# edwardyehuang/iSeg

Measured on AMD Instinct MI355X. Metric: train_images_per_sec (ConvNeXt-T+ASPP 512x512 crop, fwd+bwd+AdamW, whole job), higher is better.
Workload: dtype bf16

## Files before the change

include/iseg_hip.h:

```cpp
#ifndef ISEG_HIP_H
#define ISEG_HIP_H

#include <stddef.h>
#include <stdint.h>

#ifdef __cplusplus
extern "C" {
#endif

#ifndef ISEG_HIP_STREAM_T
#define ISEG_HIP_STREAM_T
typedef struct ihipStream_t* iseg_stream_t;
#endif

#define ISEG_STATUS_OK 0
#define ISEG_STATUS_ARG (-1)
#define ISEG_STATUS_HIP (-2)
#define ISEG_STATUS_UNSUPPORTED (-3)
#define ISEG_STATUS_WORKSPACE (-4)

#define ISEG_DTYPE_F32 0
#define ISEG_DTYPE_BF16 1

#define ISEG_ACT_NONE 0
// ... 425 lines not shown
typedef struct iseg_conv_geom {
    int N, H, W, Cin, Cout, KH, KW, sh, sw, dh, dw, pt, pl, Ho, Wo, groups;
} iseg_conv_geom;
int iseg_conv2d_igemm_supported(const iseg_conv_geom* geom_h, int dtype);
size_t iseg_conv2d_igemm_workspace_bytes(const iseg_conv_geom* geom_h, int pass);
int iseg_conv2d_igemm_fwd(const void* x, const void* w, const float* bias, void* y, const iseg_conv_geom* geom_h, int dtype, void* ws,
                          size_t ws_bytes, iseg_stream_t stream);
int iseg_conv2d_igemm_fwd_kt_supported(const iseg_conv_geom* g, int dtype);
int iseg_conv2d_igemm_fwd_kt(const void* x, const void* wt, const float* bias, void* y, const iseg_conv_geom* g, int dtype, void* ws,
                             size_t ws_bytes, iseg_stream_t stream);
int iseg_conv2d_igemm_bwd_data(const void* dy, const void* w, void* dx, const iseg_conv_geom* geom_h, int dtype, void* ws, size_t ws_bytes,
                               iseg_stream_t stream);
int iseg_conv2d_igemm_bwd_weight(const void* x, const void* dy, float* dw, int accumulate, const iseg_conv_geom* geom_h, int dtype, void* ws,
                                 size_t ws_bytes, iseg_stream_t stream);

int iseg_convnext_mlp_supported(int C, int dtype);
size_t iseg_convnext_mlp_tiled_bytes(int C, int backward);
int iseg_convnext_mlp_prep(const float* W1, const float* W2, const float* gamma, void* fw_tiled, void* bw_tiled, int C,
                           iseg_stream_t stream);
int iseg_convnext_weight_prep_batched(const int64_t* table, int entries, int64_t max_elements, iseg_stream_t stream);
int iseg_convnext_mlp_fwd(const void* y2, const void* fw_tiled, const float* b1, const float* b2, const float* gamma,
                          const float* rowscale, int64_t rows_per_group, const void* residual, void* out, int64_t M, int C, int dtype,
                          iseg_stream_t stream);
int iseg_convnext_mlp_bwd(const void* y2, const void* dbr, const void* bw_tiled, const float* b1, void* g, void* dh, void* dy2,
                          int64_t M, int C, int dtype, iseg_stream_t stream);
int iseg_convnext_mlp_bwd_data(const void* y, const float* mean, const float* rstd, const float* ln_gamma, const float* ln_beta,
                               const void* dout, const float* rowscale, int64_t rows_per_group, const void* bw_tiled, const float* b1,
                               void* dy2, int64_t M, int C, int dtype, iseg_stream_t stream);

size_t iseg_convnext_mlp_bwd_data_ln_workspace_bytes(int64_t M, int C);
// ... 18 lines not shown
```

iseg_amd/_hip.py:

```python
import ctypes as C
import os

_HERE = os.path.dirname(os.path.abspath(__file__))
LIB_PATH = os.path.join(_HERE, "lib", "libiseg_hip.so")

F32, BF16 = 0, 1
ACT_NONE, ACT_RELU, ACT_GELU, ACT_GELU_GRAD, ACT_RELU_GRAD, ACT_MUL_AUX, ACT_SIGMOID, ACT_SWISH = 0, 1, 2, 3, 4, 5, 6, 7


class HipLibraryMissing(RuntimeError):
    pass


class HipCallError(RuntimeError):
    pass


class GemmArgs(C.Structure):
    _fields_ = [
        ("A", C.c_void_p), ("lda", C.c_int64), ("a_kcontig", C.c_int),
        ("B", C.c_void_p), ("ldb", C.c_int64), ("b_kcontig", C.c_int),
        ("D", C.c_void_p), ("ldd", C.c_int64),
        ("M", C.c_int64), ("N", C.c_int64), ("K", C.c_int64),
        ("in_dtype", C.c_int), ("out_dtype", C.c_int),
# ... 2 lines not shown
        ("aux", C.c_void_p), ("ldaux", C.c_int64),
        ("pre_out", C.c_void_p), ("ldp", C.c_int64),
        ("act", C.c_int), ("alpha", C.c_float), ("accumulate", C.c_int), ("split_k", C.c_int), ("a_act", C.c_int),
        ("colsum_out", C.c_void_p), ("colsum_accumulate", C.c_int), ("defer_reduce", C.c_int),
        ("batch", C.c_int), ("batch_inner", C.c_int),
        ("sa_outer", C.c_int64), ("sa_inner", C.c_int64), ("sb_outer", C.c_int64), ("sb_inner", C.c_int64),
        ("sd_outer", C.c_int64), ("sd_inner", C.c_int64),
        ("pre_deriv", C.c_int),
        ("b_group_rows", C.c_int64),
        ("b_group_stride", C.c_int64),
    ]


class ConvGeom(C.Structure):
    _fields_ = [(n, C.c_int) for n in ("N", "H", "W", "Cin", "Cout", "KH", "KW", "sh", "sw", "dh", "dw", "pt", "pl", "Ho", "Wo", "groups")]


_p, _i, _l, _f, _z, _u64 = C.c_void_p, C.c_int, C.c_int64, C.c_float, C.c_size_t, C.c_uint64

SIGNATURES = {
    "iseg_version": (_i, []),
    "iseg_last_error": (_z, [C.c_char_p, _z]),
    "iseg_gemm_splits": (_i, [C.POINTER(GemmArgs)]),
    "iseg_gemm_tn_pair_splits": (_i, [C.POINTER(GemmArgs), C.POINTER(GemmArgs)]),
    "iseg_gemm_tn_pair": (_i, [C.POINTER(GemmArgs), _p, _z, C.POINTER(GemmArgs), _p, _z, _p]),
    "iseg_gemm_slabs": (_i, [C.POINTER(GemmArgs)]),
    "iseg_gemm_variant": (_i, [C.POINTER(GemmArgs)]),
    "iseg_gemm_workspace_bytes": (_z, [C.POINTER(GemmArgs)]),
    "iseg_gemm": (_i, [C.POINTER(GemmArgs), _p, _z, _p]),
    "iseg_gemm_reduce": (_i, [C.POINTER(GemmArgs), _p, _z, _p]),
# ... 168 lines not shown
    "iseg_augment_channel_means": (_i, [_p, _i, _p, _p, _i, _i, _i, _p, _z, _p]),
    "iseg_augment_crop_batch": (_i, [_p, _i, _p, _p, _p, C.POINTER(C.c_float), C.POINTER(C.c_float), C.POINTER(C.c_float), _i, _p, _p, _i, _i, _i,
                                     _i, _i, _u64, _p]),
    "iseg_normalize_image": (_i, [_p, _p, _l, C.POINTER(C.c_float), C.POINTER(C.c_float), _p]),
    "iseg_projective_transform_batch": (_i, [_p, _p, _p, _p, _p, _p, _i, _i, _i, _i, _i, _f, C.POINTER(C.c_float), _i, _p]),
    "iseg_upsample_ce_supported": (_i, [_i, _i, _i, _i, _i]),
    "iseg_upsample_ce_workspace_bytes": (_z, [_i, _i, _i, _i, _i, _i]),
    "iseg_upsample_ce": (_i, [_p, _i, _p, _p, _i, _i, _i, _i, _i, _i, _i, _p, _f, _p, _f, _p, _p, _z, _p]),
    "iseg_conv2d_igemm_supported": (_i, [C.POINTER(ConvGeom), _i]),
    "iseg_conv2d_igemm_workspace_bytes": (_z, [C.POINTER(ConvGeom), _i]),
    "iseg_conv2d_igemm_fwd": (_i, [_p, _p, _p, _p, C.POINTER(ConvGeom), _i, _p, _z, _p]),
    "iseg_conv2d_igemm_fwd_kt": (_i, [_p, _p, _p, _p, C.POINTER(ConvGeom), _i, _p, _z, _p]),
    "iseg_conv2d_igemm_fwd_kt_supported": (_i, [C.POINTER(ConvGeom), _i]),
    "iseg_conv2d_igemm_bwd_data": (_i, [_p, _p, _p, C.POINTER(ConvGeom), _i, _p, _z, _p]),
    "iseg_conv2d_igemm_bwd_weight": (_i, [_p, _p, _p, _i, C.POINTER(ConvGeom), _i, _p, _z, _p]),
    "iseg_convnext_mlp_supported": (_i, [_i, _i]),
    "iseg_convnext_mlp_tiled_bytes": (_z, [_i, _i]),
    "iseg_convnext_mlp_prep": (_i, [_p, _p, _p, _p, _p, _i, _p]),
    "iseg_convnext_mlp_fwd": (_i, [_p, _p, _p, _p, _p, _p, _l, _p, _p, _l, _i, _i, _p]),
    "iseg_convnext_mlp_bwd": (_i, [_p, _p, _p, _p, _p, _p, _p, _l, _i, _i, _p]),
    "iseg_convnext_mlp_bwd_data": (_i, [_p, _p, _p, _p, _p, _p, _p, _l, _p, _p, _p, _l, _i, _i, _p]),
    "iseg_convnext_mlp_bwd_data_ln_workspace_bytes": (_z, [_l, _i]),
    "iseg_convnext_mlp_bwd_data_ln": (_i, [_p, _p, _p, _p, _p, _p, _p, _l, _p, _p, _p, _p, _p, _l, _i, _i, _p, _z, _p]),
    "iseg_convnext_weight_prep_batched": (_i, [_p, _i, _l, _p]),
    "iseg_convnext_mlp_fwd_ln": (_i, [_p, _p, _p, _f, _p, _p, _p, _p, _p, _p, _p, _l, _p, _p, _l, _i, _i, _p]),
    "iseg_convnext_mlp_wgrad_workspace_bytes": (_z, [_l, _i]),
    "iseg_convnext_mlp_wgrad": (_i, [_p, _p, _p, _p, _p, _p, _p, _l, _p, _p, _p, _p, _p, _p, _p, _p, _p, _p, _l, _i, _i, _p, _z, _p]),
    "iseg_sgd_momentum_step": (_i, [_p, _p, _p, _p, _p, _p, _p, _p, _f, _i, _p, _f, _p, _f, _l, _p]),
}

# ... 35 lines not shown
```

iseg_amd/csrc/conv_igemm.hip:

```cpp
#include <type_traits>

#include "gemm_impl.h"

using namespace iseg_mm;

int gemm_reduce(const iseg_gemm_args* g, const Epi& epi, float* slabs, int eff_split, int64_t slab_rows, hipStream_t stream);

namespace {

struct ConvP {
    const bf16_t* src;
    int Hs, Ws, Cs;
    int Hr, Wr;
    int Cg;
    int kw;
    int sh, sw, dh, dw, pt, pl;
    int groups;
};

struct PhaseP {
    int Hq, Wq;
    int a, b;
    int q0h, q0w;
    int Th, Tw;
// ... 4 lines not shown
struct PhaseTable {
    PhaseP ph[MAX_PHASES];
    int H, W, sh, sw, kw;
};
struct NoPhases {};

struct PhaseRows {
    int hw, wq, H, W, sh, sw, a, b;
    __device__ __forceinline__ int64_t operator()(int64_t m) const {
        const int n = (int)(m / hw), rem = (int)(m % hw);
        return ((int64_t)n * H + (rem / wq) * sh + a) * W + (rem % wq) * sw + b;
    }
};

constexpr int INVALID = -(1 << 28);

}

#include "conv_igemm_dma.h"

namespace {

__device__ __forceinline__ bf16x8 gather8(const ConvP& p, int nb, int ih, int iw, int c, bool ok) {
    bf16x8 v;
#pragma unroll
    for (int i = 0; i < 8; ++i) v[i] = (bf16_t)0.f;
    if (ok && ih >= 0 && ih < p.Hs && iw >= 0 && iw < p.Ws) v = *reinterpret_cast<const bf16x8*>(p.src + ((int64_t)(nb + ih * p.Ws + iw)) * p.Cs + c);
    return v;
}

// ... 72 lines not shown
                const int64_t row = n0 + r;
                bf16x8 v;
#pragma unroll
                for (int u = 0; u < 8; ++u) v[u] = (bf16_t)0.f;
                if (row < R && kk < Kend) {
                    const int ij = (int)(kk / cout_g), co = (int)(kk % cout_g);
                    const int tap = tap0 + (ij / tw) * tsh + (ij % tw) * tsw;
                    v = *reinterpret_cast<const bf16x8*>(wg + tap * tap_stride + row * ld + co);
                }
                this->regs[i] = v;
            }
        }
    }
};

template <int WM, int WN, int FM, int FN, int PASS, int BK, class TO>
__global__ __launch_bounds__(WM* WN * 64) void conv_igemm_kernel(ConvP p, const bf16_t* __restrict__ Bop, int64_t ldb, int64_t b_group_stride,
                                                                  int64_t tap_stride, TO* __restrict__ D, int64_t ldd, int64_t d_group_stride,
                                                                  int64_t M, int64_t N, int64_t K, int tiles_n, int ntiles,
                                                                  int64_t k_per_split, float* __restrict__ slabs, int64_t slab_group_stride,
                                                                  Epi epi, int vecD,
                                                                  typename std::conditional<PASS == 3, PhaseTable, NoPhases>::type phases) {
    constexpr bool AKC = PASS != 2, BKC = PASS == 1 || PASS == 3;
    constexpr int GPASS = PASS == 3 ? 1 : PASS;
    constexpr int NT = WM * WN * 64;
    constexpr int BM = WM * FM * 16, BN = WN * FN * 16;
    constexpr int TM = FM * 16, TN = FN * 16;
    constexpr int KS = BK / 32;
    using GA = TileGeom<BM, AKC, BK>;
    using GB = TileGeom<BN, BKC, BK>;
    constexpr int STAGE_ELEMS = GA::elems + GB::elems;
    constexpr int EPI_BYTES = WM * WN * 32 * (TN + 4) * 4;
    constexpr int LDS_BYTES = (STAGE_ELEMS * 2 > EPI_BYTES) ? STAGE_ELEMS * 2 : EPI_BYTES;
    __shared__ __attribute__((aligned(16))) char smem[LDS_BYTES];
    bf16_t* const lds = reinterpret_cast<bf16_t*>(smem);

    const int tid = threadIdx.x, lane = tid & 63, wid = tid >> 6;
    const int wm = wid / WN, wn = wid % WN;
    const int grp = blockIdx.z;
    const int coff = grp * p.Cg;
    Bop += grp * b_group_stride;
    D += grp * d_group_stride;
    if (slabs) slabs += grp * slab_group_stride;
    if (epi.bias) epi.bias += grp * N;

    int t, ksplit;
    int tw = p.kw, tap0 = 0, tsh = p.kw, tsw = 1;
    PhaseRows rows{};
    if constexpr (PASS == 3) {
        const PhaseP& ph = phases.ph[blockIdx.y];
        M = ph.M;
        K = ph.K;
        k_per_split = K;
        t = blockIdx.x;
        ksplit = 0;
        if ((int64_t)(t / tiles_n) * BM >= M) return;
        p.Hr = ph.Hq, p.Wr = ph.Wq, p.kw = ph.Tw, p.pt = ph.q0h, p.pl = ph.q0w;
        p.sh = p.sw = p.dh = p.dw = 1;
        tw = ph.Tw, tap0 = ph.tap0, tsh = phases.sh * phases.kw, tsw = phases.sw;
        rows = PhaseRows{ph.Hq * ph.Wq, ph.Wq, phases.H, phases.W, phases.sh, phases.sw, ph.a, ph.b};
    } else {
        tile_and_split(ntiles, t, ksplit);
    }
    const int tile_n = t % tiles_n, tile_m = t / tiles_n;
    const int64_t m0 = (int64_t)tile_m * BM, n0 = (int64_t)tile_n * BN;
    const int64_t kbeg = (int64_t)ksplit * k_per_split;
    const int64_t kend = (kbeg + k_per_split < K) ? kbeg + k_per_split : K;
    const int nk = (int)((kend - kbeg + BK - 1) / BK);

    f32x4 acc[FM][FN];
#pragma unroll
    for (int i = 0; i < FM; ++i)
#pragma unroll
        for (int j = 0; j < FN; ++j) acc[i][j] = f32x4{0.f, 0.f, 0.f, 0.f};

    GatherStager<BM, NT, BK, GPASS> sa;
    typename std::conditional<BKC, TapWeightStager<BN, NT, BK>, Stager<BN, false, NT, BK>>::type sb;
    sa.prepare(p, m0, M, coff, tid);

    auto load_b = [&](int64_t k0) {
// ... 23 lines not shown
            for (int j = 0; j < FN; ++j) bfr[j] = read_frag<BN, BKC, BK>(lds + GA::elems, wn * TN + j * 16, ks, lane);
#pragma unroll
            for (int i = 0; i < FM; ++i)
#pragma unroll
                for (int j = 0; j < FN; ++j) acc[i][j] = __builtin_amdgcn_mfma_f32_16x16x32_bf16(bfr[j], af[i], acc[i][j], 0, 0, 0);
        }
        __syncthreads();
        if (more) {
            sa.store(lds, tid);
            sb.store(lds + GA::elems, tid);
            __syncthreads();
        }
    }
    if constexpr (PASS == 3) tile_epilogue<WM, WN, FM, FN, TO, PhaseRows>(acc, smem, D, ldd, M, N, m0, n0, wm, wn, wid, lane, nullptr, epi, false, vecD, 0, rows);
    else tile_epilogue<WM, WN, FM, FN, TO>(acc, smem, D, ldd, M, N, m0, n0, wm, wn, wid, lane, slabs, epi, false, vecD, ksplit);
}

struct Problem {
    int64_t M, N, K;
    ConvP p;
    const bf16_t* B;
    int64_t ldb, b_group_stride, tap_stride;
    void* D;
    int64_t ldd, d_group_stride;
    int out_dtype;
    const float* bias;
    int accumulate;
    int groups;
};

// ... 287 lines not shown
    q.M = (int64_t)g->KH * g->KW * cg;
    q.N = og;
    q.K = (int64_t)g->N * g->Ho * g->Wo;
    q.p = ConvP{(const bf16_t*)x, g->H, g->W, g->Cin, g->Ho, g->Wo, cg, g->KW, g->sh, g->sw, g->dh, g->dw, g->pt, g->pl, g->groups};
    q.B = (const bf16_t*)dy;
    q.ldb = g->Cout;
    q.b_group_stride = og;
    q.D = dw;
    q.ldd = g->Cout;
    q.d_group_stride = og;
    q.out_dtype = ISEG_F32;
    q.accumulate = accumulate;
    q.groups = g->groups;
    return run<2, float>(q, ws, ws_bytes, stream, "iseg_conv2d_igemm_bwd_weight");
}
```

iseg_amd/csrc/conv_igemm_dma.h:

```cpp
#pragma once
#include "gemm_dma.h"

namespace {

__device__ uint4 conv_zero_page[8];

template <int WM, int WN, int NS, int PASS, class TO>
__global__ __launch_bounds__(WM* WN * 64) void conv_igemm_dma_kernel(ConvP p, const bf16_t* __restrict__ Bop, int64_t ldb, int64_t tap_stride,
                                                                      TO* __restrict__ D, int64_t ldd, int64_t M, int64_t N, int64_t K,
                                                                      int tiles_n, int ntiles, int64_t k_per_split, float* __restrict__ slabs,
                                                                      Epi epi) {
    using namespace iseg_mm;
    constexpr int FN = 4;
    constexpr int NW = WM * WN;
    constexpr int BM = WM * 64, BN = WN * FN * 16;
    constexpr int PIECES = (BM + BN) / 8, PPW = PIECES / NW;
    static_assert(PIECES % NW == 0, "stage pieces must divide over the wavefronts");
    constexpr int STAGE = (BM + BN) * 128;
    extern __shared__ __attribute__((aligned(1024))) char smem[];

    const int tid = threadIdx.x, lane = tid & 63, wid = tid >> 6;
    const int wm = wid / WN, wn = wid % WN;
    int t, ksplit;
    tile_and_split(ntiles, t, ksplit);
    const int64_t m0 = (int64_t)(t / tiles_n) * BM, n0 = (int64_t)(t % tiles_n) * BN;
    const int64_t kbeg = (int64_t)ksplit * k_per_split;
    const int64_t kend = (kbeg + k_per_split < K) ? kbeg + k_per_split : K;
    const int nk = (int)((kend - kbeg) / 64);
// ... 14 lines not shown
                a1[q] = (rem % p.Wr) * p.sw - p.pl;
            } else {
                a0[q] = rem / p.Wr + p.pt;
                a1[q] = rem % p.Wr + p.pl;
            }
            a2[q] = (int64_t)n * p.Hs * p.Ws;
        } else {
            const int rb = r - BM;
            int64_t row = n0 + rb;
            row = row < N ? row : N - 1;
            a0[q] = ((lane & 7) ^ b_key(rb)) * 8;
            a1[q] = 0;
            a2[q] = row * ldb;
        }
    }
    auto issue = [&](int stage, int kt) {
        const int64_t k0 = kbeg + (int64_t)kt * 64;
        const int tap = (int)(k0 / p.Cg), c0 = (int)(k0 % p.Cg);
        const int ti = tap / p.kw, tj = tap % p.kw;
#pragma unroll
        for (int q = 0; q < PPW; ++q) {
            const int r = (wid + q * NW) * 8 + rsub;
            const bf16_t* src;
            if (r < BM) {
                const int chunk = ((lane & 7) ^ (r & 7)) * 8;
                int ih, iw;
                bool ok;
                if (PASS == 0) {
                    ih = a0[q] + ti * p.dh;
                    iw = a1[q] + tj * p.dw;
                    ok = (unsigned)ih < (unsigned)p.Hs && (unsigned)iw < (unsigned)p.Ws;
                } else {
                    const int th = a0[q] - ti * p.dh, tw = a1[q] - tj * p.dw;
                    ih = th / p.sh;
                    iw = tw / p.sw;
                    ok = th >= 0 && tw >= 0 && ih * p.sh == th && iw * p.sw == tw && ih < p.Hs && iw < p.Ws;
                }
                src = ok ? p.src + (a2[q] + (int64_t)ih * p.Ws + iw) * p.Cs + c0 + chunk : zero + chunk;
            } else if (PASS == 0) {
                src = Bop + a2[q] + k0 + a0[q];
            } else {
                src = Bop + (int64_t)tap * tap_stride + a2[q] + c0 + a0[q];
            }
            __builtin_amdgcn_global_load_lds((glb_void_ptr)src, (lds_void_ptr)(smem + stage * STAGE + (wid + q * NW) * 1024), 16, 0, 0);
        }
    };

    f32x4 acc[4][FN];
// ... 72 lines not shown
                for (int u = 0; u < 8; ++u) v[u] = acc[i][2 * h + (u >> 2)][u & 3];
                if (split) {
                    float* dst = slab + m * N + n;
                    *reinterpret_cast<float4*>(dst) = *reinterpret_cast<const float4*>(v);
                    *reinterpret_cast<float4*>(dst + 4) = *reinterpret_cast<const float4*>(v + 4);
                } else {
                    EpiPrefetch<TO> pf;
                    pf.load(epi, m, n, D, ldd);
                    epi_finish8<TO>(epi, v, pf, m, n, D, ldd);
                }
            }
        }
    }
}

}
```

iseg_amd/functional.py:

```python
import os

import torch
from torch.autograd import Function

from . import kernels as K
from . import nn
from . import dist


def _grad(p):
    if p.grad is None:
        p.grad = torch.zeros_like(p.data)
    return p.grad


def _c(t):
    return t if t.is_contiguous() else t.contiguous()


def _rows2d(t):
    C = t.shape[-1]
    if t.is_contiguous():
        return t.reshape(-1, C), C
    per16 = 16 // t.element_size()
# ... 398 lines not shown
    if groups == 1:
        return xc
    N, H, W, Cin = xc.shape
    out = torch.empty((N, H, W, Cin_g), dtype=xc.dtype, device=xc.device)
    K.copy2d(xc.reshape(-1, Cin)[:, g * Cin_g:], Cin, out.reshape(-1, Cin_g), Cin_g, N * H * W, Cin_g)
    return out


def conv2d(x, W, b=None, strides=(1, 1), dilation=(1, 1), padding="same", groups=1):
    if nn.dry_run():
        Ho, Wo, _, _ = _conv_geometry(x.shape[1], x.shape[2], W.shape[0], W.shape[1], tuple(strides), tuple(dilation), padding)
        return _dry((x.shape[0], Ho, Wo, W.shape[-1]), x, nn.compute_dtype())
    return _Conv2dFn.apply(x, W, b, tuple(strides), tuple(dilation), padding, int(groups))


class _DWConvFn(Function):
    @staticmethod
    def forward(ctx, x, W, b, dil):
        Kk, C = W.shape[0], W.shape[2]
        pad = (Kk - 1) * dil // 2
        xc = _c(x)
        y = K.dwconv2d(xc, W.data.reshape(Kk * Kk, C), b.data if b is not None else None, Kk, dil, pad, pad)
        ctx.W, ctx.b, ctx.dil, ctx.pad = W, b, dil, pad
        ctx.save_for_backward(xc)
        return y

    @staticmethod
    def backward(ctx, dy):
        (xc,) = ctx.saved_tensors
        W, b, dil, pad = ctx.W, ctx.b, ctx.dil, ctx.pad
# ... 2287 lines not shown
```

iseg_amd/kernels.py:

```python
import contextlib
import ctypes as C

import torch

from . import _hip
from ._hip import F32, BF16, ACT_NONE, ACT_RELU, ACT_GELU, ACT_GELU_GRAD, ACT_RELU_GRAD, ACT_MUL_AUX, ACT_SIGMOID, ACT_SWISH, GemmArgs

_DT = {torch.float32: F32, torch.bfloat16: BF16}


def dt(t):
    try:
        return _DT[t.dtype if isinstance(t, torch.Tensor) else t]
    except KeyError:
        raise TypeError(f"iseg_amd kernels support float32 and bfloat16 storage, got {t.dtype if isinstance(t, torch.Tensor) else t}")


def ptr(t):
    return None if t is None else t.data_ptr()


_DEVICE_INDEX = [None]


# ... 755 lines not shown
def conv2d_igemm_bwd_data(dy, w, geom):
    _require_cuda(dy, w)
    dx = torch.empty((geom.N, geom.H, geom.W, geom.Cin), dtype=dy.dtype, device=dy.device)
    ws, wsb = _conv_ws(geom, 1, dy.device)
    _hip.call("iseg_conv2d_igemm_bwd_data", ptr(dy), ptr(w), ptr(dx), C.byref(geom), dt(dy), ptr(ws), wsb, stream())
    return dx


def conv2d_igemm_bwd_weight(x, dy, dw, geom, accumulate=True):
    _require_cuda(x, dy, dw)
    ws, wsb = _conv_ws(geom, 2, x.device)
    _hip.call("iseg_conv2d_igemm_bwd_weight", ptr(x), ptr(dy), ptr(dw), int(accumulate), C.byref(geom), dt(x), ptr(ws), wsb, stream())
    return dw


def colsum(x, ldx, batch_stride, batch, rows, Cc, out, scale=1.0, accumulate=False):
    if Cc > 8192 and batch == 1 and scale == 1.0:
        L = _hip.lib()
        ws, wsb = workspace(L.iseg_colsum_wide_workspace_bytes(rows, Cc), x.device)
        _hip.check(L.iseg_colsum_wide(ptr(x), ldx, rows, Cc, ptr(out), int(accumulate), dt(x), ptr(ws), wsb, stream()), "iseg_colsum_wide")
        return out
    need = _hip.lib().iseg_colsum_workspace_bytes(batch, rows, Cc)
    ws, wsb = workspace(need, x.device)
    _hip.call("iseg_colsum", ptr(x), ldx, batch_stride, batch, rows, Cc, ptr(out), scale, int(accumulate), dt(x), ptr(ws), wsb,
              stream())
    return out


def accumulate_pair(src, n, dst0, dst1):
    if dst0 is None and dst1 is None:
# ... 892 lines not shown
```

iseg_amd/layers/aspp.py:

```python
from .. import functional as F
from ..nn import Layer
from .model_builder import ConvNormAct, ImageLevelBlock


class AtrousSpatialPyramidPooling(Layer):
    def __init__(self, filters=256, dilation_rates=[3, 6, 9], dilation_rates_multiplier=1, use_pixel_level=True,
                 use_image_level=True, name=None):
        super().__init__(name=name)
        self.filters = filters
        self.use_pixel_level = use_pixel_level
        self.use_image_level = use_image_level
        self.dilation_rates = list(dilation_rates)
        self.dilation_rates_multiplier = dilation_rates_multiplier

    def build(self, input_shape):
        if self.use_image_level:
            self.image_level_block = ImageLevelBlock(self.filters, name=f"{self.name}/image_level_block")
        if self.use_pixel_level:
            self.pixel_level_block = ConvNormAct(self.filters, (1, 1), name=f"{self.name}/pixel_level_block")
        convs = []
        for rate in self.dilation_rates:
            rate = rate * self.dilation_rates_multiplier
            convs.append(ConvNormAct(self.filters, (3, 3), dilation_rate=rate, name=f"{self.name}/asp_convs_{rate}"))
        import torch

        self.asp_convs = torch.nn.ModuleList(convs)
        self.built = True

    def call(self, inputs, training=None):
        if self._can_group(training):
            return self._call_grouped(inputs)
        branches = int(self.use_image_level) + int(self.use_pixel_level) + len(self.asp_convs)
        xs = list(F.fork(inputs, branches))
        blocks = ([self.image_level_block] if self.use_image_level else []) + ([self.pixel_level_block] if self.use_pixel_level else []) + \
            list(self.asp_convs)
        return F.concat([b(x, training=training) for b, x in zip(blocks, xs)])

    def _branch_blocks(self):
        blocks = []
        if self.use_image_level:
            blocks.append(self.image_level_block.convbnrelu)
        if self.use_pixel_level:
            blocks.append(self.pixel_level_block)
        return blocks + list(self.asp_convs)

    def _can_group(self, training):
        from .. import dist, nn
        from .base_layers import BatchNormalization

        if not (training and dist.active()) or nn.dry_run():
            return False
        for b in self._branch_blocks():
            if not (isinstance(b.bn, BatchNormalization) and b.bn.synchronized and b.bn.trainable and b.activation is F.relu and
                    b.dropout is None and b.bn.built):
                return False
        return True

    def _call_grouped(self, inputs):
        blocks = self._branch_blocks()
        xs = list(F.fork(inputs, len(blocks)))
        h, w = inputs.shape[1], inputs.shape[2]
        pre = []
        for i, b in enumerate(blocks):
            x = xs[i]
            if self.use_image_level and i == 0:
                x = F.global_avg_pool(x)
            pre.append(b.conv(x))
        outs = list(F.batch_norm_group(pre, [b.bn for b in blocks], relu=True))
        if self.use_image_level:
            outs[0] = F.broadcast_hw(outs[0], h, w)
        return F.concat(outs)
```

iseg_amd/layers/model_builder.py:

```python
import torch

from .. import functional as F
from .. import nn
from ..nn import Layer
from ..utils.common import resize_image
from .base_layers import Conv2D, Dropout, get_activation
from .normalizations import normalization


def get_training_value(training=None):
    if training is None:
        return False
    if isinstance(training, int):
        training = bool(training)
    return training


class ConvNormAct(Layer):
    def __init__(self, filters=256, kernel_size=1, dilation_rate=1, use_bn=True, activation="relu",
                 kernel_initializer="glorot_uniform", dropout_rate=0, dropout_before_bn=False, trainable=True, use_bias=False,
                 groups=1, conv_func=Conv2D, norm_func=normalization, name=None):
        super().__init__(trainable=trainable, name=name if name is not None else "ConvBnRelu")
        self.conv = conv_func(filters, kernel_size, padding="same", use_bias=use_bias, kernel_initializer=kernel_initializer,
                              dilation_rate=dilation_rate, groups=groups, trainable=trainable, name=f"{self.name}/conv")
        self.bn = None if not use_bn else norm_func(trainable=trainable, name=f"{self.name}/bn")
        self.activation = get_activation(activation)
        self.dropout = None
        self.dropout_before_bn = dropout_before_bn
        if dropout_rate > 0:
            self.dropout = Dropout(dropout_rate, name=f"{self.name}/dropout")

    def call(self, inputs, training=None):
        x = self.conv(inputs)
        should_dropout = (self.dropout is not None) and self.trainable
        if should_dropout and self.dropout_before_bn:
            x = self.dropout(x, training=training)
        act = self.activation
        if self.bn is not None:
            fuse = act is F.relu and hasattr(self.bn, "moving_mean")
            x = self.bn(x, training=training, fused_relu=True) if fuse else self.bn(x, training=training)
            if fuse:
                act = None
        if act is not None:
            x = act(x)
        if should_dropout and not self.dropout_before_bn:
            x = self.dropout(x, training=training)
        return x

# ... 134 lines not shown
```

Measured before the change: 2021.

## Fuse ASPP pixel-branch convolutions into single multi-branch igemm kernels

Adds a branch-table convolution API that runs all ASPP pixel-level and atrous convolutions sharing one input in a single kernel launch per pass. Forward launches one grid over the branches, backward-data sums all branches' taps into one joined K reduction with an optional fused residual, and backward-weight handles every branch in one launch. This is meant to cut launch count, repeated forks of the input, and separate dx accumulation across branches. The fused path only applies to bf16, bias-free, stride-1, same-padded convs with channel counts that are multiples of 64, and it adds new kernel code paths.

```diff
diff --git a/include/iseg_hip.h b/include/iseg_hip.h
--- a/include/iseg_hip.h
+++ b/include/iseg_hip.h
@@ -463,6 +463,29 @@
 int iseg_conv2d_igemm_bwd_weight(const void* x, const void* dy, float* dw, int accumulate, const iseg_conv_geom* geom_h, int dtype, void* ws,
                                  size_t ws_bytes, iseg_stream_t stream);
 
+#define ISEG_CONV_MAX_BRANCHES 4
+typedef struct iseg_conv_branch {
+    int KH, KW, dh, dw, pt, pl;
+    const void* wt;
+    const void* w;
+    const float* bias;
+    void* y;
+    int64_t ldy, y_col;
+    const void* dy;
+    int64_t lddy;
+    float* gw;
+} iseg_conv_branch;
+typedef struct iseg_conv_branches {
+    int N, H, W, Cin, Cout, count;
+    iseg_conv_branch b[ISEG_CONV_MAX_BRANCHES];
+} iseg_conv_branches;
+int iseg_conv2d_branches_supported(const iseg_conv_branches* t, int dtype);
+int iseg_conv2d_branches_fwd(const void* x, const iseg_conv_branches* t, int dtype, void* ws, size_t ws_bytes, iseg_stream_t stream);
+int iseg_conv2d_branches_bwd_data(const iseg_conv_branches* t, void* dx, const void* residual, int64_t ldr, int dtype, void* ws, size_t ws_bytes,
+                                  iseg_stream_t stream);
+int iseg_conv2d_branches_bwd_weight(const void* x, const iseg_conv_branches* t, int accumulate, int dtype, void* ws, size_t ws_bytes,
+                                    iseg_stream_t stream);
+
 int iseg_convnext_mlp_supported(int C, int dtype);
 size_t iseg_convnext_mlp_tiled_bytes(int C, int backward);
 int iseg_convnext_mlp_prep(const float* W1, const float* W2, const float* gamma, void* fw_tiled, void* bw_tiled, int C,
diff --git a/iseg_amd/_hip.py b/iseg_amd/_hip.py
--- a/iseg_amd/_hip.py
+++ b/iseg_amd/_hip.py
@@ -40,6 +40,19 @@
 
 class ConvGeom(C.Structure):
     _fields_ = [(n, C.c_int) for n in ("N", "H", "W", "Cin", "Cout", "KH", "KW", "sh", "sw", "dh", "dw", "pt", "pl", "Ho", "Wo", "groups")]
+
+
+CONV_MAX_BRANCHES = 4
+
+
+class ConvBranch(C.Structure):
+    _fields_ = [(n, C.c_int) for n in ("KH", "KW", "dh", "dw", "pt", "pl")] + [
+        ("wt", C.c_void_p), ("w", C.c_void_p), ("bias", C.c_void_p), ("y", C.c_void_p), ("ldy", C.c_int64), ("y_col", C.c_int64),
+        ("dy", C.c_void_p), ("lddy", C.c_int64), ("gw", C.c_void_p)]
+
+
+class ConvBranches(C.Structure):
+    _fields_ = [(n, C.c_int) for n in ("N", "H", "W", "Cin", "Cout", "count")] + [("b", ConvBranch * CONV_MAX_BRANCHES)]
 
 
 _p, _i, _l, _f, _z, _u64 = C.c_void_p, C.c_int, C.c_int64, C.c_float, C.c_size_t, C.c_uint64
@@ -238,6 +251,10 @@
     "iseg_conv2d_igemm_fwd_kt_supported": (_i, [C.POINTER(ConvGeom), _i]),
     "iseg_conv2d_igemm_bwd_data": (_i, [_p, _p, _p, C.POINTER(ConvGeom), _i, _p, _z, _p]),
     "iseg_conv2d_igemm_bwd_weight": (_i, [_p, _p, _p, _i, C.POINTER(ConvGeom), _i, _p, _z, _p]),
+    "iseg_conv2d_branches_supported": (_i, [C.POINTER(ConvBranches), _i]),
+    "iseg_conv2d_branches_fwd": (_i, [_p, C.POINTER(ConvBranches), _i, _p, _z, _p]),
+    "iseg_conv2d_branches_bwd_data": (_i, [C.POINTER(ConvBranches), _p, _p, _l, _i, _p, _z, _p]),
+    "iseg_conv2d_branches_bwd_weight": (_i, [_p, C.POINTER(ConvBranches), _i, _i, _p, _z, _p]),
     "iseg_convnext_mlp_supported": (_i, [_i, _i]),
     "iseg_convnext_mlp_tiled_bytes": (_z, [_i, _i]),
     "iseg_convnext_mlp_prep": (_i, [_p, _p, _p, _p, _p, _i, _p]),
diff --git a/iseg_amd/csrc/conv_igemm.hip b/iseg_amd/csrc/conv_igemm.hip
--- a/iseg_amd/csrc/conv_igemm.hip
+++ b/iseg_amd/csrc/conv_igemm.hip
@@ -42,6 +42,23 @@
 };
 
 constexpr int INVALID = -(1 << 28);
+
+struct BranchP {
+    const bf16_t* src;
+    const bf16_t* B;
+    void* D;
+    const float* bias;
+    int64_t ldb, ldd;
+    int Cs;
+    int kw, dh, dw, pt, pl;
+    int K;
+};
+constexpr int MAX_BRANCHES = ISEG_CONV_MAX_BRANCHES;
+struct BranchTable {
+    BranchP b[MAX_BRANCHES];
+    int count;
+};
+struct NoBranches {};
 
 }
 
@@ -144,13 +161,11 @@
     }
 };
 
-template <int WM, int WN, int FM, int FN, int PASS, int BK, class TO>
-__global__ __launch_bounds__(WM* WN * 64) void conv_igemm_kernel(ConvP p, const bf16_t* __restrict__ Bop, int64_t ldb, int64_t b_group_stride,
-                                                                  int64_t tap_stride, TO* __restrict__ D, int64_t ldd, int64_t d_group_stride,
-                                                                  int64_t M, int64_t N, int64_t K, int tiles_n, int ntiles,
-                                                                  int64_t k_per_split, float* __restrict__ slabs, int64_t slab_group_stride,
-                                                                  Epi epi, int vecD,
-                                                                  typename std::conditional<PASS == 3, PhaseTable, NoPhases>::type phases) {
+template <int WM, int WN, int FM, int FN, int PASS, int BK, class TO, bool RAGGED = false>
+__device__ __forceinline__ void conv_igemm_tile(ConvP p, const bf16_t* __restrict__ Bop, int64_t ldb, int64_t b_group_stride, int64_t tap_stride,
+                                                TO* __restrict__ D, int64_t ldd, int64_t d_group_stride, int64_t M, int64_t N, int64_t K, int tiles_n,
+                                                int ntiles, int64_t k_per_split, float* __restrict__ slabs, int64_t slab_group_stride, Epi epi,
+                                                int vecD, const typename std::conditional<PASS == 3, PhaseTable, NoPhases>::type& phases, int grp) {
     constexpr bool AKC = PASS != 2, BKC = PASS == 1 || PASS == 3;
     constexpr int GPASS = PASS == 3 ? 1 : PASS;
     constexpr int NT = WM * WN * 64;
@@ -167,7 +182,6 @@
 
     const int tid = threadIdx.x, lane = tid & 63, wid = tid >> 6;
     const int wm = wid / WN, wn = wid % WN;
-    const int grp = blockIdx.z;
     const int coff = grp * p.Cg;
     Bop += grp * b_group_stride;
     D += grp * d_group_stride;
@@ -194,6 +208,7 @@
     }
     const int tile_n = t % tiles_n, tile_m = t / tiles_n;
     const int64_t m0 = (int64_t)tile_m * BM, n0 = (int64_t)tile_n * BN;
+    if (RAGGED && m0 >= M) return;
     const int64_t kbeg = (int64_t)ksplit * k_per_split;
     const int64_t kend = (kbeg + k_per_split < K) ? kbeg + k_per_split : K;
     const int nk = (int)((kend - kbeg + BK - 1) / BK);
@@ -247,6 +262,26 @@
     }
     if constexpr (PASS == 3) tile_epilogue<WM, WN, FM, FN, TO, PhaseRows>(acc, smem, D, ldd, M, N, m0, n0, wm, wn, wid, lane, nullptr, epi, false, vecD, 0, rows);
     else tile_epilogue<WM, WN, FM, FN, TO>(acc, smem, D, ldd, M, N, m0, n0, wm, wn, wid, lane, slabs, epi, false, vecD, ksplit);
+}
+
+template <int WM, int WN, int FM, int FN, int PASS, int BK, class TO>
+__global__ __launch_bounds__(WM* WN * 64) void conv_igemm_kernel(ConvP p, const bf16_t* __restrict__ Bop, int64_t ldb, int64_t b_group_stride,
+                                                                  int64_t tap_stride, TO* __restrict__ D, int64_t ldd, int64_t d_group_stride,
+                                                                  int64_t M, int64_t N, int64_t K, int tiles_n, int ntiles,
+                                                                  int64_t k_per_split, float* __restrict__ slabs, int64_t slab_group_stride,
+                                                                  Epi epi, int vecD,
+                                                                  typename std::conditional<PASS == 3, PhaseTable, NoPhases>::type phases) {
+    conv_igemm_tile<WM, WN, FM, FN, PASS, BK, TO>(p, Bop, ldb, b_group_stride, tap_stride, D, ldd, d_group_stride, M, N, K, tiles_n, ntiles,
+                                                  k_per_split, slabs, slab_group_stride, epi, vecD, phases, blockIdx.z);
+}
+
+template <int WM, int WN, int FM, int FN, int BK>
+__global__ __launch_bounds__(WM* WN * 64) void conv_branches_wgrad_kernel(ConvP p, BranchTable tab, int64_t N, int64_t K, int tiles_n, int ntiles,
+                                                                           Epi epi, int vecD) {
+    const BranchP& br = tab.b[blockIdx.z];
+    p.kw = br.kw, p.dh = br.dh, p.dw = br.dw, p.pt = br.pt, p.pl = br.pl;
+    conv_igemm_tile<WM, WN, FM, FN, 2, BK, float, true>(p, br.B, br.ldb, 0, 0, (float*)br.D, br.ldd, 0, br.K, N, K, tiles_n, ntiles, K, nullptr, 0, epi,
+                                                        vecD, NoPhases{}, 0);
 }
 
 struct Problem {
@@ -564,3 +599,199 @@
     q.groups = g->groups;
     return run<2, float>(q, ws, ws_bytes, stream, "iseg_conv2d_igemm_bwd_weight");
 }
+
+namespace {
+
+bool branches_ok(const iseg_conv_branches* t) {
+    if (!t || t->count < 1 || t->count > MAX_BRANCHES || t->N <= 0 || t->H <= 0 || t->W <= 0 || t->Cin <= 0 || t->Cout <= 0) return false;
+    for (int i = 0; i < t->count; ++i) {
+        const iseg_conv_branch& b = t->b[i];
+        if (b.KH <= 0 || b.KW <= 0 || b.dh <= 0 || b.dw <= 0 || b.pt < 0 || b.pl < 0) return false;
+    }
+    return true;
+}
+
+ConvP branches_shared(const iseg_conv_branches* t, const void* src, int Cs, int Cg) {
+    return ConvP{(const bf16_t*)src, t->H, t->W, Cs, t->H, t->W, Cg, 1, 1, 1, 1, 1, 0, 0, 1};
+}
+
+struct DgradPlan {
+    bool big;
+    int nsplit;
+};
+DgradPlan branches_dgrad_plan(int64_t M, int64_t N, int64_t K) { return DgradPlan{M >= 256, conv_splits(M, N, K, 1)}; }
+
+iseg_conv_geom branches_joined_geom(const iseg_conv_branches* t) {
+    int taps = 0;
+    for (int i = 0; i < t->count; ++i) taps += t->b[i].KH * t->b[i].KW;
+    return iseg_conv_geom{t->N, t->H, t->W, t->Cin, t->Cout, 1, taps, 1, 1, 1, 1, 0, 0, t->H, t->W, 1};
+}
+
+template <int PASS, class Tile>
+void launch_branches_dma(Tile, const ConvP& p, const BranchTable& tab, int64_t ldb, int64_t tap_stride, bf16_t* D, int64_t ldd, int64_t M, int64_t N,
+                         int64_t K, int eff, int64_t kps, float* slabs, const Epi& epi, hipStream_t stream) {
+    constexpr int WM = Tile::WM, WN = Tile::WN, FN = Tile::FN, NS = Tile::NS;
+    constexpr int BM = WM * 64, BN = WN * FN * 16;
+    constexpr int lds = NS * (BM + BN) * 128;
+    const int tiles_m = (int)ceil_div64(M, BM), tiles_n = (int)ceil_div64(N, BN);
+    static const bool raised = [] {
+        return hipFuncSetAttribute(reinterpret_cast<const void*>(&conv_branches_dma_kernel<WM, WN, FN, NS, PASS>),
+                                   hipFuncAttributeMaxDynamicSharedMemorySize, lds) == hipSuccess;
+    }();
+    (void)raised;
+    hipLaunchKernelGGL((conv_branches_dma_kernel<WM, WN, FN, NS, PASS>), dim3(tiles_m * tiles_n, eff, PASS == 0 ? tab.count : 1), dim3(WM * WN * 64), lds,
+                       stream, p, tab, ldb, tap_stride, D, ldd, M, N, K, tiles_n, tiles_m * tiles_n, kps, slabs, epi);
+}
+struct BT256 { enum { WM = 4, WN = 2, FN = 4, NS = 3 }; };
+struct BT128 { enum { WM = 2, WN = 4, FN = 2, NS = 2 }; };
+
+}
+
+extern "C" int iseg_conv2d_branches_supported(const iseg_conv_branches* t, int dtype) {
+    if (!branches_ok(t) || dtype != ISEG_BF16) return 0;
+    if (t->Cin % 64 != 0 || t->Cout % 64 != 0) return 0;
+    const int64_t M = (int64_t)t->N * t->H * t->W;
+    return M >= 64 && M < (1ll << 31) / 8;
+}
+
+#define BRANCHES_COMMON(name)                                                                                                                  \
+    ISEG_REQUIRE(t, name ": null branch table");                                                                                              \
+    ISEG_REQUIRE(t->count >= 1 && t->count <= MAX_BRANCHES, name ": %d branches, the table holds 1 .. %d", t->count, MAX_BRANCHES);          \
+    ISEG_REQUIRE(branches_ok(t), name ": bad geometry");                                                                                      \
+    if (!iseg_conv2d_branches_supported(t, dtype)) {                                                                                          \
+        iseg_set_error(name ": needs bf16 storage, Cin and Cout multiples of 64 and at least 64 pixels (Cin %d, Cout %d, dtype %d)", t->Cin,  \
+                       t->Cout, dtype);                                                                                                       \
+        return ISEG_ERR_UNSUPPORTED;                                                                                                          \
+    }                                                                                                                                         \
+    const int64_t M = (int64_t)t->N * t->H * t->W
+
+extern "C" int iseg_conv2d_branches_fwd(const void* x, const iseg_conv_branches* t, int dtype, void* ws, size_t ws_bytes, hipStream_t stream) {
+    BRANCHES_COMMON("iseg_conv2d_branches_fwd");
+    (void)ws;
+    (void)ws_bytes;
+    ISEG_REQUIRE(x && ((uintptr_t)x & 15) == 0, "iseg_conv2d_branches_fwd: x must be a 16-byte aligned device pointer");
+    BranchTable tab{};
+    tab.count = t->count;
+    for (int i = 0; i < t->count; ++i) {
+        const iseg_conv_branch& b = t->b[i];
+        ISEG_REQUIRE(b.wt && b.y, "iseg_conv2d_branches_fwd: branch %d: null operand", i);
+        bf16_t* const y = (bf16_t*)b.y + b.y_col;
+        ISEG_REQUIRE((((uintptr_t)b.wt | (uintptr_t)y | (uintptr_t)b.bias) & 15) == 0 && b.ldy % 8 == 0 && b.y_col >= 0 && b.y_col + t->Cout <= b.ldy,
+                     "iseg_conv2d_branches_fwd: branch %d: operands must be 16-byte aligned, the column slice inside a row of ldy %% 8 == 0", i);
+        BranchP& d = tab.b[i];
+        d.B = (const bf16_t*)b.wt;
+        d.K = b.KH * b.KW * t->Cin;
+        d.ldb = d.K;
+        d.D = y;
+        d.ldd = b.ldy;
+        d.bias = b.bias;
+        d.kw = b.KW, d.dh = b.dh, d.dw = b.dw, d.pt = b.pt, d.pl = b.pl;
+    }
+    Epi epi{};
+    epi.alpha = 1.f;
+    epi.batch_inner = 1;
+    const ConvP p = branches_shared(t, x, t->Cin, t->Cin);
+    launch_branches_dma<0>(BT128{}, p, tab, 0, 0, nullptr, 0, M, t->Cout, 0, 1, 0, nullptr, epi, stream);
+    return iseg_check_launch("iseg_conv2d_branches_fwd");
+}
+
+extern "C" int iseg_conv2d_branches_bwd_data(const iseg_conv_branches* t, void* dx, const void* residual, int64_t ldr, int dtype, void* ws,
+                                             size_t ws_bytes, hipStream_t stream) {
+    BRANCHES_COMMON("iseg_conv2d_branches_bwd_data");
+    ISEG_REQUIRE(dx && ((uintptr_t)dx & 15) == 0, "iseg_conv2d_branches_bwd_data: dx must be a 16-byte aligned device pointer");
+    ISEG_REQUIRE(!residual || (((uintptr_t)residual & 15) == 0 && ldr % 8 == 0 && ldr >= t->Cin),
+                 "iseg_conv2d_branches_bwd_data: the residual must be 16-byte aligned with ldr %% 8 == 0");
+    BranchTable tab{};
+    tab.count = t->count;
+    int64_t K = 0;
+    for (int i = 0; i < t->count; ++i) {
+        const iseg_conv_branch& b = t->b[i];
+        ISEG_REQUIRE(b.dy && b.w, "iseg_conv2d_branches_bwd_data: branch %d: null operand", i);
+        ISEG_REQUIRE((((uintptr_t)b.dy | (uintptr_t)b.w) & 15) == 0 && b.lddy % 8 == 0 && b.lddy >= t->Cout && b.lddy < (1ll << 31),
+                     "iseg_conv2d_branches_bwd_data: branch %d: operands must be 16-byte aligned, lddy %% 8 == 0", i);
+        K += (int64_t)b.KH * b.KW * t->Cout;
+        BranchP& d = tab.b[i];
+        d.src = (const bf16_t*)b.dy;
+        d.Cs = (int)b.lddy;
+        d.B = (const bf16_t*)b.w;
+        d.K = (int)K;
+        d.kw = b.KW, d.dh = b.dh, d.dw = b.dw, d.pt = b.pt, d.pl = b.pl;
+    }
+    const int64_t N = t->Cin;
+    const DgradPlan plan = branches_dgrad_plan(M, N, K);
+    int64_t kps = K;
+    float* slabs = nullptr;
+    if (plan.nsplit > 1) {
+        const iseg_conv_geom joined = branches_joined_geom(t);
+        const size_t need = iseg_conv2d_igemm_workspace_bytes(&joined, 1);
+        ISEG_REQUIRE_WORKSPACE(ws && ws_bytes >= need, "iseg_conv2d_branches_bwd_data: split-K needs %zu workspace bytes, got %zu", need, ws_bytes);
+        slabs = (float*)ws;
+        kps = ceil_div64(ceil_div64(K, plan.nsplit), 64) * 64;
+    }
+    const int eff = (int)ceil_div64(K, kps);
+    Epi epi{};
+    epi.alpha = 1.f;
+    epi.batch_inner = 1;
+    epi.residual = residual;
+    epi.ldr = ldr;
+    const ConvP p = branches_shared(t, nullptr, 0, t->Cout);
+    const int64_t tap_stride = (int64_t)t->Cin * t->Cout;
+    if (plan.big) launch_branches_dma<1>(BT256{}, p, tab, t->Cout, tap_stride, (bf16_t*)dx, N, M, N, K, eff, kps, slabs, epi, stream);
+    else launch_branches_dma<1>(BT128{}, p, tab, t->Cout, tap_stride, (bf16_t*)dx, N, M, N, K, eff, kps, slabs, epi, stream);
+    if (!slabs) return iseg_check_launch("iseg_conv2d_branches_bwd_data");
+    iseg_gemm_args ga{};
+    ga.M = M;
+    ga.N = N;
+    ga.K = K;
+    ga.D = dx;
+    ga.ldd = N;
+    ga.in_dtype = ISEG_BF16;
+    ga.out_dtype = ISEG_BF16;
+    ga.alpha = 1.f;
+    ga.residual = residual;
+    ga.ldr = ldr;
+    return gemm_reduce(&ga, epi, slabs, eff, M, stream);
+}
+
+extern "C" int iseg_conv2d_branches_bwd_weight(const void* x, const iseg_conv_branches* t, int accumulate, int dtype, void* ws, size_t ws_bytes,
+                                               hipStream_t stream) {
+    BRANCHES_COMMON("iseg_conv2d_branches_bwd_weight");
+    (void)ws;
+    (void)ws_bytes;
+    ISEG_REQUIRE(x && ((uintptr_t)x & 15) == 0, "iseg_conv2d_branches_bwd_weight: x must be a 16-byte aligned device pointer");
+    BranchTable tab{};
+    tab.count = t->count;
+    int maxK = 0;
+    for (int i = 0; i < t->count; ++i) {
+        const iseg_conv_branch& b = t->b[i];
+        ISEG_REQUIRE(b.dy && b.gw, "iseg_conv2d_branches_bwd_weight: branch %d: null operand", i);
+        ISEG_REQUIRE((((uintptr_t)b.dy | (uintptr_t)b.gw) & 15) == 0 && b.lddy % 8 == 0 && b.lddy >= t->Cout,
+                     "iseg_conv2d_branches_bwd_weight: branch %d: operands must be 16-byte aligned, lddy %% 8 == 0", i);
+        BranchP& d = tab.b[i];
+        d.B = (const bf16_t*)b.dy;
+        d.ldb = b.lddy;
+        d.D = b.gw;
+        d.ldd = t->Cout;
+        d.K = b.KH * b.KW * t->Cin;
+        d.kw = b.KW, d.dh = b.dh, d.dw = b.dw, d.pt = b.pt, d.pl = b.pl;
+        if (d.K > maxK) maxK = d.K;
+    }
+    Epi epi{};
+    epi.alpha = 1.f;
+    epi.accumulate = accumulate;
+    epi.batch_inner = 1;
+    const ConvP p = branches_shared(t, x, t->Cin, t->Cin);
+    const int64_t N = t->Cout;
+    auto launch = [&](auto tile) {
+        constexpr int WM = decltype(tile)::WM, WN = decltype(tile)::WN, FM = decltype(tile)::FM, FN = decltype(tile)::FN;
+        constexpr int BM = WM * FM * 16, BN = WN * FN * 16;
+        const int tiles_m = (int)ceil_div64(maxK, BM), tiles_n = (int)ceil_div64(N, BN);
+        hipLaunchKernelGGL((conv_branches_wgrad_kernel<WM, WN, FM, FN, 64>), dim3(tiles_m * tiles_n, 1, tab.count), dim3(WM * WN * 64), 0, stream, p, tab,
+                           N, M, tiles_n, tiles_m * tiles_n, epi, 1);
+    };
+    struct T128 { enum { WM = 2, WN = 4, FM = 4, FN = 2 }; };
+    struct T64 { enum { WM = 4, WN = 2, FM = 2, FN = 2 }; };
+    if (N <= 64) launch(T64{});
+    else launch(T128{});
+    return iseg_check_launch("iseg_conv2d_branches_bwd_weight");
+}
diff --git a/iseg_amd/csrc/conv_igemm_dma.h b/iseg_amd/csrc/conv_igemm_dma.h
--- a/iseg_amd/csrc/conv_igemm_dma.h
+++ b/iseg_amd/csrc/conv_igemm_dma.h
@@ -5,13 +5,14 @@
 
 __device__ uint4 conv_zero_page[8];
 
-template <int WM, int WN, int NS, int PASS, class TO>
-__global__ __launch_bounds__(WM* WN * 64) void conv_igemm_dma_kernel(ConvP p, const bf16_t* __restrict__ Bop, int64_t ldb, int64_t tap_stride,
-                                                                      TO* __restrict__ D, int64_t ldd, int64_t M, int64_t N, int64_t K,
-                                                                      int tiles_n, int ntiles, int64_t k_per_split, float* __restrict__ slabs,
-                                                                      Epi epi) {
+template <int WM, int WN, int NS, int PASS, class TO, class Tab, int FN = 4>
+__device__ __forceinline__ void conv_igemm_dma_tile(ConvP p, const bf16_t* __restrict__ Bop, int64_t ldb, int64_t tap_stride, TO* __restrict__ D,
+                                                    int64_t ldd, int64_t M, int64_t N, int64_t K, int tiles_n, int ntiles, int64_t k_per_split,
+                                                    float* __restrict__ slabs, const Epi& epi, const Tab& tab) {
     using namespace iseg_mm;
-    constexpr int FN = 4;
+    constexpr bool JOINED = std::is_same<Tab, BranchTable>::value;
+    static_assert(!JOINED || PASS == 1, "only the data gradient joins its branches along K");
+    static_assert(FN == 2 || FN == 4, "a wavefront's tile is 64 rows by 32 or 64 columns");
     constexpr int NW = WM * WN;
     constexpr int BM = WM * 64, BN = WN * FN * 16;
     constexpr int PIECES = (BM + BN) / 8, PPW = PIECES / NW;
@@ -56,8 +57,27 @@
             a2[q] = row * ldb;
         }
     }
+    int bi = 0;
+    int64_t bk0 = 0, bk1 = K;
+    auto enter = [&](int64_t k0) {
+        if constexpr (JOINED) {
+            while (bi + 1 < tab.count && k0 >= tab.b[bi].K) ++bi;
+            const BranchP& br = tab.b[bi];
+            bk0 = bi ? tab.b[bi - 1].K : 0;
+            bk1 = br.K;
+            p.src = br.src, p.Cs = br.Cs, p.kw = br.kw, p.dh = br.dh, p.dw = br.dw, p.pt = br.pt, p.pl = br.pl;
+            Bop = br.B;
+        }
+    };
+    enter(kbeg);
     auto issue = [&](int stage, int kt) {
-        const int64_t k0 = kbeg + (int64_t)kt * 64;
+        int64_t k0 = kbeg + (int64_t)kt * 64;
+        int pt = 0, pl = 0;
+        if constexpr (JOINED) {
+            if (k0 >= bk1) enter(k0);
+            k0 -= bk0;
+            pt = p.pt, pl = p.pl;
+        }
         const int tap = (int)(k0 / p.Cg), c0 = (int)(k0 % p.Cg);
         const int ti = tap / p.kw, tj = tap % p.kw;
 #pragma unroll
@@ -73,7 +93,7 @@
                     iw = a1[q] + tj * p.dw;
                     ok = (unsigned)ih < (unsigned)p.Hs && (unsigned)iw < (unsigned)p.Ws;
                 } else {
-                    const int th = a0[q] - ti * p.dh, tw = a1[q] - tj * p.dw;
+                    const int th = a0[q] + pt - ti * p.dh, tw = a1[q] + pl - tj * p.dw;
                     ih = th / p.sh;
                     iw = tw / p.sw;
                     ok = th >= 0 && tw >= 0 && ih * p.sh == th && iw * p.sw == tw && ih < p.Hs && iw < p.Ws;
@@ -176,4 +196,29 @@
     }
 }
 
-}
+template <int WM, int WN, int NS, int PASS, class TO>
+__global__ __launch_bounds__(WM* WN * 64) void conv_igemm_dma_kernel(ConvP p, const bf16_t* __restrict__ Bop, int64_t ldb, int64_t tap_stride,
+                                                                      TO* __restrict__ D, int64_t ldd, int64_t M, int64_t N, int64_t K,
+                                                                      int tiles_n, int ntiles, int64_t k_per_split, float* __restrict__ slabs,
+                                                                      Epi epi) {
+    conv_igemm_dma_tile<WM, WN, NS, PASS, TO>(p, Bop, ldb, tap_stride, D, ldd, M, N, K, tiles_n, ntiles, k_per_split, slabs, epi, NoBranches{});
+}
+
+template <int WM, int WN, int FN, int NS, int PASS>
+__global__ __launch_bounds__(WM* WN * 64) void conv_branches_dma_kernel(ConvP p, BranchTable tab, int64_t ldb, int64_t tap_stride,
+                                                                         bf16_t* __restrict__ D, int64_t ldd, int64_t M, int64_t N, int64_t K,
+                                                                         int tiles_n, int ntiles, int64_t k_per_split, float* __restrict__ slabs,
+                                                                         Epi epi) {
+    if constexpr (PASS == 0) {
+        const BranchP& br = tab.b[blockIdx.z];
+        p.kw = br.kw, p.dh = br.dh, p.dw = br.dw, p.pt = br.pt, p.pl = br.pl;
+        epi.bias = br.bias;
+        conv_igemm_dma_tile<WM, WN, NS, 0, bf16_t, NoBranches, FN>(p, br.B, br.ldb, 0, (bf16_t*)br.D, br.ldd, M, N, br.K, tiles_n, ntiles, br.K,
+                                                                   nullptr, epi, NoBranches{});
+    } else {
+        conv_igemm_dma_tile<WM, WN, NS, 1, bf16_t, BranchTable, FN>(p, nullptr, ldb, tap_stride, D, ldd, M, N, K, tiles_n, ntiles, k_per_split, slabs,
+                                                                    epi, tab);
+    }
+}
+
+}
diff --git a/iseg_amd/functional.py b/iseg_amd/functional.py
--- a/iseg_amd/functional.py
+++ b/iseg_amd/functional.py
@@ -436,6 +436,64 @@
     return _Conv2dFn.apply(x, W, b, tuple(strides), tuple(dilation), padding, int(groups))
 
 
+def _branch_taps(Ws, dilations):
+    return [(W.shape[0], W.shape[1], d[0], d[1]) for W, d in zip(Ws, dilations)]
+
+
+def conv2d_branches_supported(x, Ws, dilations):
+    from . import _hip
+
+    cdt = nn.compute_dtype()
+    if not (torch.is_tensor(x) and x.is_cuda and x.dim() == 4 and x.dtype == cdt and 1 <= len(Ws) <= _hip.CONV_MAX_BRANCHES):
+        return False
+    N, H, Wd, Cin = x.shape
+    Cout = Ws[0].shape[3]
+    if any(W is None or W.dim() != 4 or W.shape[2] != Cin or W.shape[3] != Cout for W in Ws):
+        return False
+    if not K.conv2d_branches_supported(K.conv_branches(N, H, Wd, Cin, Cout, _branch_taps(Ws, dilations)), cdt):
+        return False
+    return all(nn.wt(W, (W.shape[0] * W.shape[1] * Cin, Cout)) is not None for W in Ws)
+
+
+class _Conv2dBranchesFn(Function):
+
+    @staticmethod
+    def forward(ctx, x, dilations, *Ws):
+        N, H, Wd, Cin = x.shape
+        Cout = Ws[0].shape[3]
+        xc = _c(x)
+        ctx.taps = _branch_taps(Ws, dilations)
+        table = K.conv_branches(N, H, Wd, Cin, Cout, ctx.taps)
+        ys = K.conv2d_branches_fwd(xc, [nn.wt(W, (W.shape[0] * W.shape[1] * Cin, Cout)) for W in Ws], table)
+        ctx.Ws = Ws
+        ctx.save_for_backward(xc)
+        return tuple(ys)
+
+    @staticmethod
+    def backward(ctx, *dys):
+        (xc,) = ctx.saved_tensors
+        Ws = ctx.Ws
+        N, H, Wd, Cin = xc.shape
+        Cout = Ws[0].shape[3]
+        rows = [_rows2d(dy) for dy in dys]
+        dy2, ld = [r[0] for r in rows], [r[1] for r in rows]
+        live = [i for i, W in enumerate(Ws) if W.requires_grad]
+        if live:
+            table = K.conv_branches(N, H, Wd, Cin, Cout, [ctx.taps[i] for i in live])
+            K.conv2d_branches_bwd_weight(xc, [dy2[i] for i in live], [ld[i] for i in live], [_grad(Ws[i]) for i in live], table, accumulate=True)
+        dx = None
+        if ctx.needs_input_grad[0]:
+            dx = K.conv2d_branches_bwd_data(dy2, ld, [nn.w(W) for W in Ws], K.conv_branches(N, H, Wd, Cin, Cout, ctx.taps))
+        for W in Ws:
+            dist.grads_ready(W, None)
+        return (dx, None) + (None,) * len(Ws)
+
+
+def conv2d_branches(x, Ws, dilations):
+    _check_act_dtype(x)
+    return list(_Conv2dBranchesFn.apply(x, tuple(tuple(d) for d in dilations), *Ws))
+
+
 class _DWConvFn(Function):
     @staticmethod
     def forward(ctx, x, W, b, dil):
diff --git a/iseg_amd/kernels.py b/iseg_amd/kernels.py
--- a/iseg_amd/kernels.py
+++ b/iseg_amd/kernels.py
@@ -793,6 +793,51 @@
     return dw
 
 
+def conv_branches(N, H, W, Cin, Cout, taps):
+    t = _hip.ConvBranches(N, H, W, Cin, Cout, len(taps))
+    for b, (kh, kw, dh, dw) in zip(t.b, taps[:_hip.CONV_MAX_BRANCHES]):
+        b.KH, b.KW, b.dh, b.dw = kh, kw, dh, dw
+        b.pt, b.pl = same_pad(H, kh, 1, dh)[1], same_pad(W, kw, 1, dw)[1]
+    return t
+
+
+def conv2d_branches_supported(table, dtype):
+    return dtype in _DT and bool(_hip.lib().iseg_conv2d_branches_supported(C.byref(table), _DT[dtype]))
+
+
+def conv_branches_joined_geom(table):
+    taps = sum(b.KH * b.KW for b in table.b[:table.count])
+    return conv_geom(table.N, table.H, table.W, table.Cin, table.Cout, 1, taps, 1, 1, 1, 1, 0, 0, table.H, table.W, 1)
+
+
+def conv2d_branches_fwd(x, wts, table, biases=None):
+    _require_cuda(x, *wts)
+    ys = [torch.empty((table.N, table.H, table.W, table.Cout), dtype=x.dtype, device=x.device) for _ in wts]
+    for i, (b, wt, y) in enumerate(zip(table.b, wts, ys)):
+        b.wt, b.y, b.ldy, b.y_col = ptr(wt), ptr(y), table.Cout, 0
+        b.bias = ptr(biases[i]) if biases is not None else None
+    _hip.call("iseg_conv2d_branches_fwd", ptr(x), C.byref(table), dt(x), None, 0, stream())
+    return ys
+
+
+def conv2d_branches_bwd_data(dys, lddys, ws_, table, residual=None):
+    _require_cuda(*dys, *ws_)
+    dx = torch.empty((table.N, table.H, table.W, table.Cin), dtype=dys[0].dtype, device=dys[0].device)
+    for b, dy, ld, w in zip(table.b, dys, lddys, ws_):
+        b.dy, b.lddy, b.w = ptr(dy), ld, ptr(w)
+    ws, wsb = _conv_ws(conv_branches_joined_geom(table), 1, dx.device)
+    _hip.call("iseg_conv2d_branches_bwd_data", C.byref(table), ptr(dx), ptr(residual), table.Cin, dt(dx), ptr(ws), wsb, stream())
+    return dx
+
+
+def conv2d_branches_bwd_weight(x, dys, lddys, gws, table, accumulate=True):
+    _require_cuda(x, *dys, *gws)
+    for b, dy, ld, gw in zip(table.b, dys, lddys, gws):
+        b.dy, b.lddy, b.gw = ptr(dy), ld, ptr(gw)
+    _hip.call("iseg_conv2d_branches_bwd_weight", ptr(x), C.byref(table), int(accumulate), dt(x), None, 0, stream())
+    return gws
+
+
 def colsum(x, ldx, batch_stride, batch, rows, Cc, out, scale=1.0, accumulate=False):
     if Cc > 8192 and batch == 1 and scale == 1.0:
         L = _hip.lib()
diff --git a/iseg_amd/layers/aspp.py b/iseg_amd/layers/aspp.py
--- a/iseg_amd/layers/aspp.py
+++ b/iseg_amd/layers/aspp.py
@@ -30,11 +30,37 @@
     def call(self, inputs, training=None):
         if self._can_group(training):
             return self._call_grouped(inputs)
+        pixel = self._pixel_blocks()
+        if self._convs_as_one_node(inputs, pixel):
+            xs = list(F.fork(inputs, int(self.use_image_level) + 1))
+            outs = [self.image_level_block(xs[0], training=training)] if self.use_image_level else []
+            pre = self._pixel_convs(xs[-1], pixel)
+            return F.concat(outs + [b.norm_act(y, training=training) for b, y in zip(pixel, pre)])
         branches = int(self.use_image_level) + int(self.use_pixel_level) + len(self.asp_convs)
         xs = list(F.fork(inputs, branches))
         blocks = ([self.image_level_block] if self.use_image_level else []) + ([self.pixel_level_block] if self.use_pixel_level else []) + \
             list(self.asp_convs)
         return F.concat([b(x, training=training) for b, x in zip(blocks, xs)])
+
+    def _pixel_blocks(self):
+        return ([self.pixel_level_block] if self.use_pixel_level else []) + list(self.asp_convs)
+
+    def _convs_as_one_node(self, inputs, blocks):
+        from .. import nn
+        from .base_layers import Conv2D
+
+        if nn.dry_run() or len(blocks) < 2:
+            return False
+        for b in blocks:
+            c = b.conv
+            if not (isinstance(c, Conv2D) and c.built and c.bias is None and c.activation is None and c.groups == 1 and
+                    tuple(c.strides) == (1, 1) and c.padding == "same"):
+                return False
+        return F.conv2d_branches_supported(inputs, [b.conv.kernel for b in blocks], [b.conv.dilation_rate for b in blocks])
+
+    @staticmethod
+    def _pixel_convs(x, blocks):
+        return F.conv2d_branches(x, [b.conv.kernel for b in blocks], [b.conv.dilation_rate for b in blocks])
 
     def _branch_blocks(self):
         blocks = []
@@ -58,14 +84,20 @@
 
     def _call_grouped(self, inputs):
         blocks = self._branch_blocks()
-        xs = list(F.fork(inputs, len(blocks)))
         h, w = inputs.shape[1], inputs.shape[2]
-        pre = []
-        for i, b in enumerate(blocks):
-            x = xs[i]
-            if self.use_image_level and i == 0:
-                x = F.global_avg_pool(x)
-            pre.append(b.conv(x))
+        pixel = self._pixel_blocks()
+        if self._convs_as_one_node(inputs, pixel):
+            xs = list(F.fork(inputs, int(self.use_image_level) + 1))
+            pre = [blocks[0].conv(F.global_avg_pool(xs[0]))] if self.use_image_level else []
+            pre += self._pixel_convs(xs[-1], pixel)
+        else:
+            xs = list(F.fork(inputs, len(blocks)))
+            pre = []
+            for i, b in enumerate(blocks):
+                x = xs[i]
+                if self.use_image_level and i == 0:
+                    x = F.global_avg_pool(x)
+                pre.append(b.conv(x))
         outs = list(F.batch_norm_group(pre, [b.bn for b in blocks], relu=True))
         if self.use_image_level:
             outs[0] = F.broadcast_hw(outs[0], h, w)
diff --git a/iseg_amd/layers/model_builder.py b/iseg_amd/layers/model_builder.py
--- a/iseg_amd/layers/model_builder.py
+++ b/iseg_amd/layers/model_builder.py
@@ -31,7 +31,9 @@
             self.dropout = Dropout(dropout_rate, name=f"{self.name}/dropout")
 
     def call(self, inputs, training=None):
-        x = self.conv(inputs)
+        return self.norm_act(self.conv(inputs), training=training)
+
+    def norm_act(self, x, training=None):
         should_dropout = (self.dropout is not None) and self.trainable
         if should_dropout and self.dropout_before_bn:
             x = self.dropout(x, training=training)
```

Result: faster. 2053, median of 6 (+1.6%).
